# aditya-v-kallappa/FInCFlow

Hardware: AMD Instinct MI355X
Metric: inverse images/sec (+ fwd+logdet ms/img in `forward`), 3x3 conv @64x64x96 (higher is better)
Workload: dtype f32

## Files before the change

### fincflow_amd/csrc/finc_mfma.hip

```cpp
#include "finc_common.h"
#include "finc_tile.h"

#include <stdlib.h>

#include <mutex>
#include <type_traits>
#include <utility>
#include <vector>

namespace {

typedef float v4f __attribute__((ext_vector_type(4)));
typedef unsigned v2u __attribute__((ext_vector_type(2)));
typedef unsigned v4u __attribute__((ext_vector_type(4)));

template <int CQP_, int KH_, int KW_, int NW_ = 1>
struct Cfg {
    static constexpr int CQP = CQP_, KH = KH_, KW = KW_, NW = NW_;
    static constexpr int MTB = CQP / 16;
    static constexpr int NSM = (CQP % 16) / 4;
    static constexpr int MT = MTB + NSM;
    static constexpr int NKZT = CQP / 4;
    static constexpr int NKDT = CQP / 4;
    static_assert(NW == 1 || (NKZT % NW == 0 && NKDT % NW == 0), "K-split must divide the k-steps and the output registers");
// ... 104 lines not shown
    } while (0)
#else
#define FINC_STAMP_AT(k) do { } while (0)
#endif

__device__ unsigned finc_hlp_timeouts = 0;
__device__ unsigned *finc_fault_word = nullptr;
#ifndef FINC_HLP_BUDGET_LOG2
#define FINC_HLP_BUDGET_LOG2 20
#endif
#ifdef FINC_HLP_COUNT
__device__ unsigned finc_hlp_late[2] = {0, 0};
#define FINC_HLP_LATE(k) do { if ((threadIdx.x & 63) == 0) atomicAdd(&finc_hlp_late[k], 1u); } while (0)
extern "C" int finc_debug_hlp_late(unsigned *h) { return (int)hipMemcpyFromSymbol(h, HIP_SYMBOL(finc_hlp_late), 8); }
#else
#define FINC_HLP_LATE(k) do { } while (0)
#endif

constexpr unsigned OFF_INVALID = 0x80000000u;
constexpr unsigned OFF_BAD_CHANNEL = 0x40000000u;

template <int CQP, int KH, int KW, bool SEC, int NW = 1, int NPW = 1, int S64 = 0, int HLP = 0, bool ZPRE = false>
__global__ __launch_bounds__(HLP ? 512 : 64 * NW * NPW) void finc_wave_kernel(const float *__restrict__ in,
                                                            const float *__restrict__ packed, float *__restrict__ out,
                                                            int G, int CQ, int H, int W, int P, int Tend,
                                                            unsigned orient)
{
    using C = Cfg<CQP, KH, KW, NW>;
    constexpr int MT = C::MT, NKZ = C::NKZ, NKD = C::NKD, NK = C::NK, NFRAG = C::NFRAG;
    constexpr int JS = 4 * (KH - 1);
    constexpr int SS = NK * JS;
    extern __shared__ __attribute__((aligned(16))) float lds[];
    static_assert(!HLP || (S64 == 3 && NW == 1 && NPW == 1), "helper waves: the sector-pairing kernel, one compute wave per problem");
    static_assert(!ZPRE || HLP, "premultiplied input: the helper-wave form only");
    const int wvt = (HLP || NW * NPW > 1) ? __builtin_amdgcn_readfirstlane(threadIdx.x >> 6) : 0;
    const bool helper = HLP && wvt >= 4;
    const int wv = HLP ? 0 : wvt % NW;
    const int prob = HLP ? (wvt & 3) : wvt / NW;
    const int lane = threadIdx.x & 63;
    const int q = lane >> 4, p = lane & 15;
    const int bg = blockIdx.x * (HLP ? 4 : NPW) + prob;
    const int g = bg % G;
    const unsigned o = finc_group_orient(orient, g);
    const bool fh = (o & FINC_FLIP_H) != 0, fw = (o & FINC_FLIP_W) != 0;
    const int HW = H * W;
    const unsigned slab_bytes = (unsigned)CQ * (unsigned)HW * 4u;
    const int bg_in = bg, bg_out = bg;
    const __amdgpu_buffer_rsrc_t rin =
        __builtin_amdgcn_make_buffer_rsrc((void *)(in + (size_t)bg_in * CQ * HW), 0, (int)slab_bytes, 0x00020000);
    const __amdgpu_buffer_rsrc_t rout =
        __builtin_amdgcn_make_buffer_rsrc((void *)(out + (size_t)bg_out * CQ * HW), 0, (int)slab_bytes, 0x00020000);
    const int D = W - P + 1;
    const int fifo_n = D * SS;
    const int wave_lds = C::ZRING + C::XRING + fifo_n + SS + 64;
    float *const lds_p = lds + prob * (C::XCH + NW * wave_lds);
    float *xch = lds_p;
    float *zring = lds_p + C::XCH + wv * wave_lds;
    float *xring = zring + C::ZRING;
    auto zcell = [](int qq, int rr) {
        const int lo = ((rr >> 2) ^ ((0x3200 >> (4 * (rr & 3))) & 3)) | ((qq & 1) << 2);
        return lo | (((rr & 3) | ((qq >> 1) << 2)) << 3);
    };
    float *fifo = xring + C::XRING;
    const int trash = fifo_n + lane;
    const unsigned flag_a = (unsigned)(uintptr_t)(lds + 4 * wave_lds + 4 * prob);
    auto flag_set = [flag_a](auto word_c, int v) {
        constexpr int WORD = decltype(word_c)::value;
        (void)flag_a;
#ifdef FINC_HLP_INJECT_TIMEOUT
        if (WORD == 1 && v >= 8) return;
#endif
        if constexpr (HLP) asm volatile("ds_write_b32 %0, %1 offset:%2" ::"v"(flag_a), "v"(v), "n"(4 * WORD) : "memory");
    };
    auto flag_peek = [flag_a](auto word_c, int &reg) {
        constexpr int WORD = decltype(word_c)::value;
        (void)flag_a;
        if constexpr (HLP) asm volatile("ds_read_b32 %0, %1 offset:%2" : "=v"(reg) : "v"(flag_a), "n"(4 * WORD) : "memory");
    };
    auto flag_wait = [flag_a](auto word_c, int target) {
        constexpr int WORD = decltype(word_c)::value;
#ifndef FINC_HLP_NOWAIT
#define FINC_HLP_NOWAIT 0
#endif
        if constexpr (HLP && !((FINC_HLP_NOWAIT >> WORD) & 1)) {
            int budget = 1 << FINC_HLP_BUDGET_LOG2;
            for (; budget > 0; --budget) {
                int v;
                asm volatile("ds_read_b32 %0, %1 offset:%2\n\ts_waitcnt lgkmcnt(0)" : "=v"(v) : "v"(flag_a), "n"(4 * WORD) : "memory");
                if (__builtin_amdgcn_readfirstlane(v) >= target) break;
                __builtin_amdgcn_s_sleep(2);
            }
            if (budget == 0 && (threadIdx.x & 63) == 0) {
                atomicAdd(&finc_hlp_timeouts, 1u);
                if (finc_fault_word) __hip_atomic_store(finc_fault_word, 1u, __ATOMIC_RELAXED, __HIP_MEMORY_SCOPE_SYSTEM);
            }
        }
    };

    constexpr int NSMALL = (NFRAG / MT) * C::NSM, NSR = (NSMALL + 3) / 4;
    float af[NFRAG];
    float afs[NSR > 0 ? NSR : 1];
    constexpr bool PAIR2 = finc_pair2_form<C>(HLP);
    constexpr int NPAIRF = PAIR2 ? C::NPAIR : C::NPAIR1;
    float afp[C::PAIR ? NPAIRF : 1];
    static_assert(!C::PAIR || ((NKZ * C::NSM) % 4 == 0 && (NK * C::NSM) % 4 == 0),
                  "a packed block register must not straddle a paired and an unpaired tap");
    auto small_paired = [](int sfr) {
        const int tapi = sfr < NKZ * C::NSM ? 0 : 1 + (sfr - NKZ * C::NSM) / (NK * (C::NSM > 0 ? C::NSM : 1));
        return C::PAIR && ((tapi >= 1 && tapi <= 4) || (PAIR2 && (tapi == 6 || tapi == 7)));
    };
    if (!helper) {
        const float *pk = packed + (size_t)g * C::NPACK * 64 + lane;
        auto gindex = [&](int f) {
            if (f < NKZ * MT) return (wv * NKZ + f / MT) * MT + f % MT;
            const int ff = f - NKZ * MT;
            return C::NKZT * MT + ((ff / (MT * NKD)) * C::NKDT + wv * NKD + (ff / MT) % NKD) * MT + ff % MT;
        };
#pragma unroll
        for (int f = 0; f < NFRAG; ++f) {
            if (f % MT >= C::MTB) continue;
            if (ZPRE && f < NKZ * MT) { af[f] = 0.f; continue; }
            if (NW == 1 && f < NKZ * MT && finc_zterm_is_zero(C::MTB, f / MT, f % MT)) { af[f] = 0.f; continue; }
            af[f] = pk[gindex(f) * 64];
        }
        const int quad = (lane & 15) >> 2;
#pragma unroll
        for (int r = 0; r < NSR; ++r) {
            if (small_paired(4 * r)) { afs[r] = 0.f; continue; }
            int gi = 0;
#pragma unroll
            for (int a = 3; a >= 0; --a) {
                const int sfr = 4 * r + a < NSMALL ? 4 * r + a : NSMALL - 1;
                constexpr int NSMD = C::NSM > 0 ? C::NSM : 1;
                const int f = (sfr / NSMD) * MT + C::MTB + sfr % NSMD;
                const int ga = gindex(f);
                gi = (a == 3 || quad == a) ? ga : gi;
            }
            afs[r] = pk[gi * 64];
        }
#pragma unroll
        for (int f = 0; f < NFRAG; ++f) {
            if (f % MT >= C::MTB) continue;
            if (ZPRE && f < NKZ * MT) continue;
            if (NW == 1 && f < NKZ * MT && finc_zterm_is_zero(C::MTB, f / MT, f % MT)) continue;
            asm volatile("" : "+a"(af[f]));
        }
#pragma unroll
        for (int r = 0; r < NSR; ++r) {
            if (small_paired(4 * r)) continue;
            asm volatile("" : "+a"(afs[r]));
        }
        if constexpr (C::PAIR) {
            const float *pp = packed + finc_pair_offset(G, C::NPACK, C::NPAIR, g, 0) + lane;
#pragma unroll
            for (int f = 0; f < NPAIRF; ++f) afp[f] = pp[f * 64];
#pragma unroll
            for (int f = 0; f < NPAIRF; ++f) asm volatile("" : "+a"(afp[f]));
        }
    }
    auto mma = [&](v4f &acc_, int f, float b) {
        const int mt = f % MT;
        if (mt < C::MTB) acc_ = __builtin_amdgcn_mfma_f32_16x16x4f32(af[f], b, acc_, 0, 0, 0);
        else {
            const int sfr = (f / MT) * C::NSM + (mt - C::MTB);
            finc_mma_small(acc_, afs[sfr >> 2], b, sfr & 3);
        }
    };
    v4f bias[MT];
    {
        const float *pb = packed + ((size_t)g * C::NPACK + C::NFRAGT + (wv == 0 ? 0 : 4 * MT)) * 64 + lane;
#pragma unroll
        for (int mt = 0; mt < MT; ++mt)
            bias[mt] = (v4f){pb[(4 * mt + 0) * 64], pb[(4 * mt + 1) * 64], pb[(4 * mt + 2) * 64], pb[(4 * mt + 3) * 64]};
    }
    for (int i = lane; i < fifo_n + SS + 64; i += 64) fifo[i] = 0.f;

    const int fl4 = -((p + 3) >> 2);
    const int k0 = fw ? 3 : 0, k1 = fw ? 2 : 1, k2 = fw ? 1 : 2, k3 = fw ? 0 : 3;
    const unsigned lane_t = 4u * (unsigned)q * HW * 4u, lane_b = (unsigned)q * HW * 4u;
    unsigned cmask[NKD];
#pragma unroll
    for (int j = 0; j < NKD; ++j) cmask[j] = chan_d(C::MTB, wv * NKD + j, q) < CQ ? 0u : OFF_BAD_CHANNEL;
    const unsigned zlast = (4 * (wv * NKZ + NKZ - 1) + q) < CQ ? 0u : OFF_BAD_CHANNEL;
    unsigned zpad[NW > 1 ? NKZ : 1];
    if constexpr (NW > 1) {
#pragma unroll
        for (int j = 0; j < NKZ; ++j) zpad[j] = (4 * (wv * NKZ + j) + q) < CQ ? 0u : OFF_BAD_CHANNEL;
    }
    auto zmark = [&](int j) { return NW > 1 ? zpad[j] : (j == NKZ - 1 ? zlast : 0u); };
    const int rowstep = (fh ? -P : P) * W * 4;
    const int dirw = fw ? -1 : 1;

    constexpr unsigned long long PARTNER = 0xCBAFED8943276501ull;
    const int cls = ((p + 3) >> 2) & 1;
    const int part = (int)((PARTNER >> (4 * p)) & 15);
    int srvrow[2], srvhalf[2];
#pragma unroll
    for (int wp = 0; wp < 2; ++wp) {
        const bool own = cls == wp || p >= P;
        srvrow[wp] = own ? p : part;
        srvhalf[wp] = own ? 0 : 1;
    }
    int lcolS[2], lrowS[2], loffS[2], lslotS[2], ldst[2];
    int scolS[2], srowS[2], soffS[2];
#pragma unroll
    for (int wp = 0; wp < 2; ++wp) {
        const int R = srvrow[wp], h = srvhalf[wp];
        const int f = -((R + 3) >> 2);
        lcolS[wp] = 4 * ((wp ? -3 : -4) + 4 + f);
        lrowS[wp] = R;
        lslotS[wp] = ((4 * (((wp ? -3 : -4) + 2 + f + h) % 3 + 3)) % 12);
        ldst[wp] = 4 * zcell(q, R);
        const int c = lcolS[wp] + 4 * h;
        loffS[wp] = ((fh ? H - 1 - R : R) * W + (fw ? W - 4 - c : c)) * 4 + (4 * wv * NKZ + q) * HW * 4;
        scolS[wp] = 4 * ((wp ? -1 : 0) - 2 + f);
        srowS[wp] = R;
        const int sc = scolS[wp] + 4 * h;
        soffS[wp] = ((fh ? H - 1 - R : R) * W + (fw ? W - 4 - sc : sc)) * 4;
    }
    v4u Z[2][NKZ];
#pragma unroll
    for (int wp = 0; wp < 2; ++wp)
#pragma unroll
        for (int j = 0; j < NKZ; ++j) Z[wp][j] = (v4u){0u, 0u, 0u, 0u};
    float XS[2][NKD][4];
#pragma unroll
    for (int wp = 0; wp < 2; ++wp)
#pragma unroll
// ... 73 lines not shown
            if ((FINC_S64_ABLATE & 4) == 0 && phi == 0) {
                const bool ok = lcolS[WP] >= 0 && lrowS[WP] < H && p < P;
                const unsigned vl = ok ? (unsigned)loffS[WP] : OFF_INVALID;
                const unsigned vu = ok ? (unsigned)(loffS[WP] + 32 * dirw) : OFF_INVALID;
#pragma unroll
                for (int j = 0; j < NKZ; ++j) {
                    unsigned ol = j == NKZ - 1 ? vl + zlast : vl, ou = j == NKZ - 1 ? vu + zlast : vu;
                    int so = __builtin_amdgcn_readfirstlane(j * 16 * HW);
                    if constexpr (ZPRE) {
                        const bool tile = j < 4 * C::MTB;
                        const bool last_group = tile ? (C::NSM == 0 && (j >> 2) == C::MTB - 1) : j == C::NKDT - 1;
                        const unsigned add = (tile ? lane_t - lane_b : 0u) + ((last_group && C::CQP != CQ) ? cmask[j] : 0u);
                        ol = vl + add; ou = vu + add;
                        so = __builtin_amdgcn_readfirstlane((tile ? 16 * (j >> 2) + (j & 3) : 16 * C::MTB + 4 * (j - 4 * C::MTB)) * HW * 4);
                    }
                    if constexpr (ZA_AGPR)
                        asm volatile("buffer_load_dwordx4 %0, %1, %2, %3 offen" : "=a"(ZA[WP][j]) : "v"(ol), "s"(rin), "s"(so) : "memory");
                    else
                        asm volatile("buffer_load_dwordx4 %0, %1, %2, %3 offen" : "=v"(Z[WP][j]) : "v"(ol), "s"(rin), "s"(so) : "memory");
                    asm volatile("buffer_load_dwordx4 %0, %1, %2, %3 offen" : "=a"(ZU[WP][j]) : "v"(ou), "s"(rin), "s"(so) : "memory");
                }
            }
            lcolS[WP] += 8;
            loffS[WP] += 32 * dirw;
            if (lcolS[WP] == W) { lcolS[WP] = 0; lrowS[WP] += P; loffS[WP] += rowstep - dirw * W * 4; }
        }
    };

    auto s64_event = [&](auto wp_c, auto vm_c, int pub_b = -0x7fffffff) { s64_part(wp_c, vm_c, pub_b, IC<0>{}); };

    auto sec_event = [&](auto wp_c) {
        constexpr int WP = decltype(wp_c)::value;
        if constexpr (!SEC) return;
        if constexpr (S64L) return;
        float *dst = zring + lslotS[WP] * 64 + ldst[WP];
#pragma unroll
        for (int j = 0; j < NKZ; ++j) *reinterpret_cast<v4u *>(dst + j * C::ZSLOTS * 64) = Z[WP][j];
        lslotS[WP] = lslotS[WP] >= 4 ? lslotS[WP] - 4 : lslotS[WP] + 8;
        const bool ok = lcolS[WP] >= 0 && lrowS[WP] < H && p < P;
        const unsigned vb = ok ? (unsigned)loffS[WP] : OFF_INVALID;
#pragma unroll
        for (int j = 0; j < NKZ; ++j)
            Z[WP][j] = __builtin_amdgcn_raw_buffer_load_b128(rin, (NW > 1 || j == NKZ - 1) ? vb + zmark(j) : vb, j * 16 * HW, 0);
        lcolS[WP] += 8;
        loffS[WP] += 32 * dirw;
        if (lcolS[WP] == W) { lcolS[WP] = 0; lrowS[WP] += P; loffS[WP] += rowstep - dirw * W * 4; }
    };
    auto sec_sread = [&](auto wp_c, int pub_b2 = -0x7fffffff) {
        constexpr int WP = decltype(wp_c)::value;
        if constexpr (!SEC) return;
        if (cls != WP && p < P) {
#pragma unroll
            for (int j = 0; j < NKD; ++j) {
                const float *xo = xring + j * C::XSLOTS * 64, *xp = xring + j * C::XSLOTS * 64;
                XS[WP ^ 1][j][0] = xo[xown[0]];
                XS[WP ^ 1][j][1] = xo[xown[1]];
                XS[WP ^ 1][j][2] = xo[xown[2]];
                XS[WP ^ 1][j][3] = xo[xown[3]];
                XS[WP][j][0] = xp[xprt[0]];
                XS[WP][j][1] = xp[xprt[1]];
                XS[WP][j][2] = xp[xprt[2]];
                XS[WP][j][3] = xp[xprt[3]];
            }
        }
        if constexpr (HLP) {
            if (pub_b2 != -0x7fffffff) {
                asm volatile("s_waitcnt lgkmcnt(0)" ::: "memory");
                flag_set(IC<2>{}, pub_b2);
            }
        }
        const bool ok = scolS[WP] >= 0 && srowS[WP] < H && p < P;
        st_off = ok ? (unsigned)soffS[WP] : OFF_INVALID;
        if constexpr (S64S) {
            const int phi = ((scolS[WP] + 64) >> 3) & 1;
            spark = phi == 0;
            st_off2 = (ok && phi == 1) ? (unsigned)(soffS[WP] - 32 * dirw) : OFF_INVALID;
            if (phi == 0) st_off = OFF_INVALID;
        }
        scolS[WP] += 8;
        soffS[WP] += 32 * dirw;
        if (scolS[WP] == W) { scolS[WP] = 0; srowS[WP] += P; soffS[WP] += rowstep - dirw * W * 4; }
    };
    auto sec_swrite = [&](auto wp_c, int j0, int j1) {
        constexpr int WP = decltype(wp_c)::value;
        if constexpr (!SEC) return;
        const unsigned vt = st_off == OFF_INVALID ? OFF_INVALID : st_off + lane_t;
        const unsigned vb = st_off == OFF_INVALID ? OFF_INVALID : st_off + lane_b;
        const int cpad = C::CQP - CQ;
#pragma unroll
        for (int j = 0; j < NKD; ++j) {
            if (j < j0 || j >= j1) continue;
            const int jj = wv * NKD + j;
            const bool tile = jj < 4 * C::MTB;
            const int uni = __builtin_amdgcn_readfirstlane((tile ? 16 * (jj >> 2) + (jj & 3) : 16 * C::MTB + 4 * (jj - 4 * C::MTB)) * HW * 4);
            unsigned vo = tile ? vt : vb;
            const bool last_group = tile ? (C::NSM == 0 && (jj >> 2) == C::MTB - 1) : jj == C::NKDT - 1;
            if ((NW > 1 || last_group) && cpad != 0) vo += cmask[j];
            v4u v;
            v.x = __builtin_bit_cast(unsigned, XS[WP][j][0]);
            v.y = __builtin_bit_cast(unsigned, XS[WP][j][1]);
            v.z = __builtin_bit_cast(unsigned, XS[WP][j][2]);
            v.w = __builtin_bit_cast(unsigned, XS[WP][j][3]);
            if constexpr (S64S) {
                const unsigned vo2 = st_off2 == OFF_INVALID ? OFF_INVALID : vo - st_off + st_off2;
                if constexpr (PK_AGPR && (!HLP || WP == 0)) {
                    asm volatile("buffer_store_dwordx4 %0, %1, %2, %3 offen" ::"a"(PK[WP][j]), "v"(vo2), "s"(rout), "s"(uni) : "memory");
                } else {
// ... 108 lines not shown
            if constexpr (PH == 1 && !(AB & 2)) io_swrite(0, S1);
            if constexpr (PH == 2) {
                if constexpr (!(AB & 2)) io_swrite(S1, S2);
                if constexpr (!(AB & 4)) io_land();
                if constexpr (!(AB & 1)) io_issue(0, L1, false);
            }
            if constexpr (PH == 3) {
                if constexpr (!(AB & 2)) io_swrite(S2, NKD);
                if constexpr (!(AB & 1)) io_issue(L1, NKZ, true);
            }
        }
    };

    constexpr bool ROT = (KH - 1 + KW) < 6;
    float Q[KH][4][NK];
    float R[KH][KW][NK];
    float DL[KH][KH][NK];
#pragma unroll
    for (int a = 0; a < KH; ++a) {
#pragma unroll
        for (int k = 0; k < 4; ++k)
#pragma unroll
            for (int j = 0; j < NK; ++j) Q[a][k][j] = 0.f;
#pragma unroll
        for (int b = 0; b < KW; ++b)
#pragma unroll
            for (int j = 0; j < NK; ++j) R[a][b][j] = 0.f;
#pragma unroll
        for (int k = 0; k < KH; ++k)
#pragma unroll
            for (int j = 0; j < NK; ++j) DL[a][k][j] = 0.f;
    }
    float fv[KH][NK];
#pragma unroll
    for (int a = 0; a < KH; ++a)
#pragma unroll
        for (int j = 0; j < NK; ++j) fv[a][j] = 0.f;

    const int push_l = p - (P - (KH - 1));
    const bool do_push = KH > 1 && push_l >= 0 && p < P;
    const int push_base = do_push ? q * (KH - 1) + push_l : trash;
    const int push_stride = do_push ? SS : 0;
    int pop_base[KH], pop_stride[KH];
#pragma unroll
    for (int a = 1; a < KH; ++a) {
        pop_base[a] = p < a ? q * (KH - 1) + (KH - 1 - a + p) : trash;
        pop_stride[a] = p < a ? SS : 0;
    }
    int fslot = 0;
    float *push_p = fifo + push_base;
    float *pop_p[KH];
#pragma unroll
    for (int a = 1; a < KH; ++a) pop_p[a] = fifo + pop_base[a] + (D > 1 ? pop_stride[a] : 0);
    auto fifo_push = [&](const float (&v)[NK]) {
#pragma unroll
        for (int j = 0; j < NK; ++j) push_p[j * JS] = v[j];
    };
    auto fifo_pop_all = [&]() {
#pragma unroll
        for (int a = 1; a < KH; ++a) {
#pragma unroll
            for (int j = 0; j < NK; ++j) fv[a][j] = pop_p[a][j * JS];
        }
    };
    auto fifo_advance = [&]() {
        ++fslot;
        push_p += push_stride;
#pragma unroll
        for (int a = 1; a < KH; ++a) pop_p[a] += pop_stride[a];
        if (__builtin_expect(fslot == D, 0)) {
            FINC_COLD();
            fslot = 0;
            push_p = fifo + push_base;
        }
        if (__builtin_expect(fslot + 1 == D, 0)) {
            FINC_COLD();
#pragma unroll
            for (int a = 1; a < KH; ++a) pop_p[a] = fifo + pop_base[a];
        }
    };
    auto shift_all = [&](const float (&src)[NK], auto ph_c) {
        constexpr int PHX = decltype(ph_c)::value;
        if constexpr (KH > 1) {
            float sn[KH][NK];
            ShiftOp<1>::apply(sn[1], fv[1], src);
            if constexpr (KH > 2) ShiftOp<2>::apply(sn[2], fv[2], src);
            if constexpr (KH > 3) ShiftOp<3>::apply(sn[3], fv[3], src);
            if constexpr (KH > 4) ShiftOp<4>::apply(sn[4], fv[4], src);
            if constexpr (KH > 5) ShiftOp<5>::apply(sn[5], fv[5], src);
            if constexpr (KH > 6) ShiftOp<6>::apply(sn[6], fv[6], src);
            if constexpr (ROT) {
#pragma unroll
                for (int a = 1; a < KH; ++a)
#pragma unroll
                    for (int j = 0; j < NK; ++j) Q[a][PHX][j] = sn[a][j];
            } else {
#pragma unroll
                for (int j = 0; j < NK; ++j) R[1][0][j] = sn[1][j];
#pragma unroll
                for (int a = 2; a < KH; ++a) {
#pragma unroll
                    for (int k = a - 2; k >= 1; --k)
#pragma unroll
                        for (int j = 0; j < NK; ++j) DL[a][k][j] = DL[a][k - 1][j];
#pragma unroll
                    for (int j = 0; j < NK; ++j) DL[a][0][j] = sn[a][j];
                }
            }
        }
    };

    if constexpr (HLP) {
        if (!helper) { flag_set(IC<0>{}, 0); flag_set(IC<1>{}, -1); flag_set(IC<2>{}, 0); flag_set(IC<3>{}, 0); }
    }
    __syncthreads();

    if constexpr (HLP) {
        if (helper) {
            s64_init();
            const int wlast = Tend >> 2;
            s64_event(IC<0>{}, IC<0>{});
            s64_event(IC<1>{}, IC<0>{});
            s64_event(IC<0>{}, IC<0>{});
            sec_sread(IC<1>{});
            sec_swrite(IC<1>{}, 0, NKD);
            s64_event(IC<1>{}, IC<0>{}, 0);
            sec_sread(IC<0>{});
            asm volatile("s_waitcnt lgkmcnt(0)" ::: "memory");
            flag_set(IC<2>{}, 1);
            sec_swrite(IC<0>{}, 0, NKD);
            constexpr int VMS = 1 + 2 * NKD + 2 * NKZ + 2 * NKD;
// ... 50 lines not shown
        for (int mt = 0; mt < MT; ++mt) acc[mt] = (v4f){0.f, 0.f, 0.f, 0.f};
        float zqc[C::NSM > 0 ? C::NSM : 1], zqn[C::NSM > 0 ? C::NSM : 1];
#pragma unroll
        for (int sb = 0; sb < (C::NSM > 0 ? C::NSM : 1); ++sb) zqc[sb] = zqn[sb] = 0.f;
        v4f accp = (v4f){0.f, 0.f, 0.f, 0.f};
        v4f accq = (v4f){0.f, 0.f, 0.f, 0.f};
        float cy[2] = {0.f, 0.f};

        auto phase_a = [&](auto pha_c, int j0, int j1) {
            constexpr int PHA = decltype(pha_c)::value;
#pragma unroll
            for (int j = j0; j < j1; ++j)
#pragma unroll
                for (int mt = 0; mt < (C::PAIR ? C::MTB : MT); ++mt) {
                    if constexpr (KW > 1)
                        mma(acc[mt], FT + ((0 * KW + 1 - 1) * NK + j) * MT + mt, ROT ? Q[0][(PHA + 3) & 3][j] : R[0][1][j]);
                    if constexpr (KH > 1)
                        mma(acc[mt], FT + ((1 * KW + 0 - 1) * NK + j) * MT + mt, ROT ? Q[1][(PHA + 3) & 3][j] : R[1][0][j]);
                }
            if constexpr (C::PAIR) {
#pragma unroll
                for (int j = j0; j < j1; ++j) {
                    accp = __builtin_amdgcn_mfma_f32_16x16x4f32(afp[j], Q[0][(PHA + 3) & 3][j], accp, 0, 0, 0);
                    accp = __builtin_amdgcn_mfma_f32_16x16x4f32(afp[NK + j], Q[1][(PHA + 3) & 3][j], accp, 0, 0, 0);
                }
            }
        };

#ifdef FINC_STAMP
        unsigned stamp_acc[40];
#pragma unroll
        for (int i = 0; i < 40; ++i) stamp_acc[i] = 0u;
        unsigned long long stamp_prev = 0;
        bool stamp_on = false;
#endif
        auto step = [&](auto ph_c, auto wp_c) {
            constexpr int PH = decltype(ph_c)::value;
            FINC_STAMP_AT(9);
            std::conditional_t<C::PAIR, int, bool> wrap_state;
            if constexpr (C::PAIR) wrap_state = (tm - P) & ~tm;
            else wrap_state = tm >= 0 && tm < P;
            auto any_wrap = [&]() -> bool {
                if constexpr (C::PAIR) {
                    asm volatile("" : "+s"(wrap_state));
                    return wrap_state < 0;
                } else {
                    return wrap_state;
                }
            };
            const bool any_idle = tp1 < P - 1;
            float zraw[NKZ], zv[NKZ], xpk[NKD];
            float xown[NKD];
            v4f accn[MT];
            if constexpr (HLP && PH == 0) {
                asm volatile("s_waitcnt lgkmcnt(0)" ::: "memory");
                if (__builtin_expect(__builtin_amdgcn_readfirstlane(peek_b) < win, 0)) { FINC_COLD(); FINC_HLP_LATE(0); flag_wait(IC<1>{}, win); }
            }
            if constexpr (HLP && PH == 1) flag_peek(IC<2>{}, peek_b2);
            if constexpr (C::PAIR) {
                float rs[C::NSM];
#pragma unroll
                for (int sb = 0; sb < C::NSM; ++sb) {
                    rs[sb] = finc_block_reduce(acc[C::MTB + sb]);
                    if constexpr (ZPRE) rs[sb] += zqc[sb];
                }
                if constexpr (PAIR2) {
                    accp = accq;
                    accp.x += cy[0] + rs[0];
                    accp.y += cy[1] + rs[1];
                } else {
                    const float c0 = accp.z, c1 = accp.w;
                    accp = (v4f){c0 + rs[0], c1 + rs[1], 0.f, 0.f};
                }
            }

#pragma unroll
            for (int j = 0; j < NKZ; ++j) zraw[j] = FINC_ABLATE >= 3 ? af[j] : zrd[j * C::ZSLOTS * 64];
            if constexpr (!ROT) {
#pragma unroll
                for (int a = 0; a < KH; ++a) {
#pragma unroll
                    for (int b = KW - 1; b >= 1; --b) {
                        if (a + b >= 2) {
#pragma unroll
                            for (int j = 0; j < NK; ++j) R[a][b][j] = R[a][b - 1][j];
                        }
                    }
                    if (a >= 2) {
#pragma unroll
                        for (int j = 0; j < NK; ++j) R[a][0][j] = DL[a][a - 2][j];
                    }
                }
                if (__builtin_expect(any_wrap(), 0)) {
                    FINC_COLD();
                    const bool wrapn = p == tm;
#pragma unroll
                    for (int a = 0; a < KH; ++a)
#pragma unroll
                        for (int b = 1; b < KW; ++b) {
                            if (a + b >= 2) {
#pragma unroll
                                for (int j = 0; j < NK; ++j) R[a][b][j] = wrapn ? 0.f : R[a][b][j];
                            }
                        }
                }
            }
// ... 81 lines not shown

            auto post1 = [&]() {
                if constexpr (FINC_ABLATE >= 2 && NW == 1) {
                    pack_d<C>(acc, xpk);
#pragma unroll
                    for (int j = 0; j < NKD; ++j) asm volatile("" ::"v"(xpk[j]));
                    return;
                }
                if constexpr (C::PAIR) {
#pragma unroll
                    for (int mt = 0; mt < C::MTB; ++mt) {
                        xpk[4 * mt + 0] = acc[mt].x;
                        xpk[4 * mt + 1] = acc[mt].y;
                        xpk[4 * mt + 2] = acc[mt].z;
                        xpk[4 * mt + 3] = acc[mt].w;
                    }
                    xpk[4 * C::MTB + 0] = accp.x;
                    xpk[4 * C::MTB + 1] = accp.y;
                    if constexpr (PAIR2) {
                        cy[0] = accp.z;
                        cy[1] = accp.w;
                    }
                    if (__builtin_expect(any_wrap(), 0)) {
                        FINC_COLD();
                        const bool wrapn = p == tm;
                        const float c0 = accp.z, c1 = accp.w;
                        if constexpr (PAIR2) {
                            cy[0] = wrapn ? 0.f : c0;
                            cy[1] = wrapn ? 0.f : c1;
                        } else {
                            accp.z = wrapn ? 0.f : c0;
                            accp.w = wrapn ? 0.f : c1;
                        }
                    }
                } else if constexpr (NW == 1) {
                    pack_d<C>(acc, xpk);
                    if constexpr (ZPRE) {
#pragma unroll
                        for (int sb = 0; sb < C::NSM; ++sb) xpk[4 * C::MTB + sb] += zqc[sb];
                    }
                } else {
#pragma unroll
                    for (int j = 0; j < NKD; ++j) {
                        float sum = xown[j];
#pragma unroll
                        for (int src = 0; src < NW; ++src)
                            if (src != wv)
                                sum += C::XALIAS ? xring[j * C::XSLOTS * 64 + PH * 64 + xwin]
                                                 : xch[((wv * NW + src) * NKD + j) * 64 + lane];
                        xpk[j] = sum;
                    }
                }
#pragma unroll
                for (int j = 0; j < NKD; ++j) xring[j * C::XSLOTS * 64 + PH * 64 + xwin] = xpk[j];
                if constexpr (KH > 1) {
                    fifo_push(xpk);
                    fifo_pop_all();
                }
                if constexpr (C::PAIR) {
#pragma unroll
                    for (int j = 0; j < NK; ++j) Q[0][PH][j] = xpk[j];
                } else if constexpr (KW > 1) {
                    if (__builtin_expect(any_wrap(), 0)) {
                        FINC_COLD();
                        const bool wrapn = p == tm;
#pragma unroll
                        for (int j = 0; j < NK; ++j) (ROT ? Q[0][PH][j] : R[0][1][j]) = wrapn ? 0.f : xpk[j];
                    } else {
#pragma unroll
                        for (int j = 0; j < NK; ++j) (ROT ? Q[0][PH][j] : R[0][1][j]) = xpk[j];
                    }
                }
            };
            auto post2 = [&]() {
                if constexpr (FINC_ABLATE < 2) shift_all(xpk, ph_c);
                if constexpr (C::PAIR && FINC_ABLATE < 2) {
                    if (__builtin_expect(any_wrap(), 0)) {
                        FINC_COLD();
                        const bool wrapn = p == tm;
#pragma unroll
                        for (int j = 0; j < NK; ++j) Q[0][PH][j] = wrapn ? 0.f : Q[0][PH][j];
                    }
                }
            };

            auto chunk = [&](auto ci_c) {
                constexpr int CI = decltype(ci_c)::value;
                constexpr int a = BT::a_of(CI), b = BT::b_of(CI);
#pragma unroll
                for (int j = 0; j < NK; ++j)
#pragma unroll
                    for (int mt = 0; mt < ((C::PAIR && ((a + b == 2 && a < 2) || (PAIR2 && a == 2 && b < 2))) ? C::MTB : MT); ++mt)
                        mma(accn[mt], FT + ((a * KW + b - 1) * NK + j) * MT + mt, ROT ? Q[a][(PH + 9 - a - b) & 3][j] : R[a][b][j]);
                if constexpr (PAIR2 && a == 2 && b == 0) {
#pragma unroll
                    for (int j = 0; j < NK; ++j)
                        accq = __builtin_amdgcn_mfma_f32_16x16x4f32(afp[2 * NK + j], Q[2][(PH + 7) & 3][j], j == 0 ? (v4f){0.f, 0.f, 0.f, 0.f} : accq, 0, 0, 0);
                }
                if constexpr (CI == 0) {
                    if constexpr (HLP && PH == 1) {
                        asm volatile("s_waitcnt lgkmcnt(0)" ::: "memory");
                        if (__builtin_expect(__builtin_amdgcn_readfirstlane(peek_b2) < win + 1, 0)) { FINC_COLD(); FINC_HLP_LATE(1); flag_wait(IC<2>{}, win + 1); }
                    }
                    post1();
                    if constexpr (HLP && PH == 3) flag_set(IC<0>{}, win + 1);
                }
                if constexpr (!HLP && CI == (NCH > 1 ? 1 : 0)) io_phase(ph_c, wp_c);
                if constexpr (CI == (NCH > 2 ? 2 : NCH - 1)) {
                    post2();
                    if constexpr (HLP && PH == 3) flag_peek(IC<1>{}, peek_b);
                }
                FINC_SB();
                if constexpr (CI < 6) FINC_STAMP_AT(2 + CI);
            };
            if constexpr (NCH == 0) {
                post1();
                io_phase(ph_c, wp_c);
                post2();
                FINC_SB();
            } else {
                [&]<int... I>(std::integer_sequence<int, I...>) { (chunk(IC<I>{}), ...); }
                (std::make_integer_sequence<int, NCH>{});
            }
#pragma unroll
            for (int mt = 0; mt < MT; ++mt) acc[mt] = accn[mt];
            if constexpr (ZPRE) {
#pragma unroll
                for (int sb = 0; sb < C::NSM; ++sb) zqc[sb] = zqn[sb];
            }
            if constexpr (NW > 1) __syncthreads();
            ++tp1;
            ++tm; if (tm == W) tm = 0;
            ++nslot; zrd += zstep[PH];
            if (nslot == 12) { nslot = 0; zrd -= 12 * 64; }
            if constexpr (PH == 3) { xwin ^= 256; ++win; }
            fifo_advance();
            FINC_STAMP_AT(8);
        };

        if constexpr (HLP) {
        } else if constexpr (SEC) {
            sec_sread(IC<1>{});
            sec_swrite(IC<1>{}, 0, NKD);
            sec_event(IC<1>{});
            s64_event(IC<1>{}, IC<0>{});
        } else {
            io_sread();
            io_swrite(0, NKD);
            io_land();
            io_issue(0, NKZ, true);
        }
#pragma unroll
        for (int k = 0; k < 3; ++k) {
            ++tp1; ++tm;
            ++nslot; zrd += zstep[k];
            if (nslot == 12) { nslot = 0; zrd -= 12 * 64; }
            fifo_advance();
        }
        {
            const bool started = p <= tp1;
            flag_wait(IC<1>{}, 0);
            peek_b = 0;
#pragma unroll
            for (int mt = 0; mt < MT; ++mt) {
                const float b0 = bias[mt].x, b1 = bias[mt].y, b2 = bias[mt].z, b3 = bias[mt].w;
                acc[mt] = (v4f){started ? b0 : 0.f, started ? b1 : 0.f, started ? b2 : 0.f, started ? b3 : 0.f};
                if constexpr (ZPRE) acc[mt] = (v4f){0.f, 0.f, 0.f, 0.f};
            }
#pragma unroll
            for (int j = 0; j < NKZ; ++j) {
                const float v = zrd[j * C::ZSLOTS * 64];
                const float zvj = started ? v : 0.f;
                if constexpr (ZPRE) {
                    if (j < 4 * C::MTB) acc[j >> 2][j & 3] = zvj;
                    else zqc[j - 4 * C::MTB] = zvj;
                    continue;
                }
#pragma unroll
                for (int mt = 0; mt < MT; ++mt) {
                    if (NW == 1 && finc_zterm_is_zero(C::MTB, j, mt)) continue;
                    mma(acc[mt], FZ + j * MT + mt, zvj);
                }
            }
            ++tp1; ++tm;
            ++nslot; zrd += zstep[3];
            if (nslot == 12) { nslot = 0; zrd -= 12 * 64; }
            xwin ^= 256;
            fifo_advance();
        }
        for (int t0 = 0; t0 < Tend; t0 += SEC ? 8 : 4) {
#ifdef FINC_STAMP
            stamp_on = t0 >= 64 && t0 < 192;
#endif
            step(IC<0>{}, IC<0>{});
            step(IC<1>{}, IC<0>{});
            step(IC<2>{}, IC<0>{});
            step(IC<3>{}, IC<0>{});
            if constexpr (SEC) {
                step(IC<0>{}, IC<1>{});
                step(IC<1>{}, IC<1>{});
                step(IC<2>{}, IC<1>{});
                step(IC<3>{}, IC<1>{});
            }
        }
        if constexpr (HLP) {
        } else if constexpr (SEC) {
            sec_sread(IC<0>{});
            sec_swrite(IC<0>{}, 0, NKD);
        } else {
            io_sread();
            io_swrite(0, NKD);
        }
#ifdef FINC_STAMP
        if (blockIdx.x == 517 && threadIdx.x == 0) {
#pragma unroll
            for (int i = 0; i < 40; ++i) finc_stamp_buf[i] = stamp_acc[i];
        }
#endif
    }
}

__global__ void pack_kernel(const float *__restrict__ wc, const float *__restrict__ scale,
                            const float *__restrict__ shift, float *__restrict__ packed, int Cq, int KH, int KW, int MT,
                            int NKZ, int NKD, int MTB, int nfrag, int npair)
{
    extern __shared__ __attribute__((aligned(16))) double sm[];
    const int g = blockIdx.x;
    const float *wg = wc + (size_t)g * Cq * Cq * KH * KW;
    const int KK = KH * KW;
    double *Linv = sm;
    const int npack = nfrag + 8 * MT;
    for (int j = threadIdx.x; j < Cq; j += blockDim.x) {
        for (int r = 0; r < Cq; ++r) {
            double s = (r == j) ? 1.0 : 0.0;
            for (int k = j; k < r; ++k) s -= (double)wg[((size_t)r * Cq + k) * KK + (KK - 1)] * Linv[k * Cq + j];
            Linv[r * Cq + j] = (r < j) ? 0.0 : s;
        }
    }
    __syncthreads();
    for (int e = threadIdx.x; e < nfrag * 64; e += blockDim.x) {
        const int lane = e & 63, f = e >> 6;
// ... 248 lines not shown
    size_t bank_offset = 0;
    int tail_images = 0;
    bool zpre = false;
    bool affine = false;
    bool align16 = true;
    FincSplitPlan split{};
};

static InvForm inverse_form(int Cq, int H, int W, int KH, int KW)
{
    if (finc_big_bank(Cq, KH, KW)) return finc_big_supported(Cq, H, W, KH, KW) ? INV_BIG : INV_NONE;
    if (stream_bank(Cq, KH, KW)) return finc_stream_supported(Cq, H, W, KH, KW, true) ? INV_STREAM : INV_NONE;
    if (W % 4 != 0 || W < 4 || H < 1) return INV_NONE;
    const int P = W < 16 ? W : 16;
    if (P < KH - 1) return INV_NONE;
    if (!find_inst(padded_cq(Cq, KH, KW), KH, KW, -1, W))
        return finc_big_wide_bank(Cq, KH, KW) && finc_big_supported(Cq, H, W, KH, KW) ? INV_WIDE : INV_NONE;
    if ((size_t)Cq * H * W * 4 >= ((size_t)1 << 30)) return INV_NONE;
    return INV_TABLE;
}

static InvPlan inverse_plan(const FincShape &s)
{
    InvPlan p;
    p.form = inverse_form(s.Cq, s.H, s.W, s.KH, s.KW);
    if (p.form == INV_NONE) return p;
    p.affine = p.form != INV_BIG && p.form != INV_WIDE;
    if (p.form == INV_WIDE) p.bank_offset = wave_bank_bytes(s.G, s.Cq, s.KH, s.KW);
    if (p.form == INV_BIG || p.form == INV_WIDE) return p;
    p.split = finc_split_plan(s);
    p.align16 = !p.split.takes;
    if (p.form == INV_STREAM) return p;

    const long long problems = (long long)s.B * s.G;
    const int cqp = padded_cq(s.Cq, s.KH, s.KW), P = s.W < 16 ? s.W : 16;
    const Inst *i = find_inst(cqp, s.KH, s.KW, problems, s.W);
    if (!i) return InvPlan{};
    if (i->nw == 1 && i->npw == 1 && problems % 2 == 0) {
        const Inst *k = nullptr;
        if (borrowed_cqp(cqp, s.KH, s.KW) && borrowed_form_wins(problems, lds_bytes(*i, s.W, P)))
            k = pair_inst(borrowed_cqp(cqp, s.KH, s.KW), s.KH, s.KW, s.W);
        if (!k && 4 * lds_bytes(*i, s.W, P) + 64 > 160 * 1024) k = pair_inst(cqp, s.KH, s.KW, s.W);
        if (k) i = k;
    }
    p.inst = i;
    if (p.split.takes) {
        p.form = INV_SPLIT;
        return p;
    }
    if (i == borrowed_inst(s.Cq, s.KH, s.KW))
        p.bank_offset = bank_bytes(bank_inst(s.Cq, s.KH, s.KW), s.G);
    const size_t lds = lds_bytes(*i, s.W, P);
    const bool s64 = s.W % 16 == 0 && i->fn_s64 && !finc_no_s64();
    const bool hlp = s64 && i->fn_hlp && problems % 4 == 0 && 4 * lds + 64 <= 160 * 1024 && !finc_no_hlp();
    p.io = hlp ? 3 : s64 ? 2 : s.W % 8 == 0 ? 1 : 0;
    p.fn = hlp ? i->fn_hlp : s64 ? i->fn_s64 : s.W % 8 == 0 ? i->fn_sec : i->fn;
    p.lds = hlp ? 4 * lds + 64 : lds;
    p.grid = hlp ? s.B * s.G / 4 : s.B * s.G / i->npw;
    p.block = hlp ? 512 : 64 * i->nw * i->npw;

    static const bool no_remainder = finc_env("FINC_NO_REMAINDER_LAUNCH") != nullptr;
    const bool one_wave = i->nw == 1 && i->npw == 1, packed_pair = i->nw == 2 && i->npw == 2;
    if (!no_remainder && (one_wave || packed_pair)) {
        long long n1 = packed_pair ? 2 : hlp ? 4 : (long long)((160 * 1024 - 64) / lds);
        n1 = n1 > 4 ? 4 : n1 < 1 ? 1 : n1;
        const long long round = n1 * 256, r = problems % round;
        if (problems > round && r != 0 && r <= 512 && r % s.G == 0) {
            FincShape tail = s;
            tail.B = (int)(r / s.G);
            const InvPlan t = inverse_plan(tail);
            if (t.form == INV_SPLIT || t.inst != i) p.tail_images = tail.B;
        }
    }
    p.zpre = hlp && i->fn_zpre && p.tail_images == 0;
    return p;
}

bool finc_mfma_supported(int Cq, int H, int W, int KH, int KW) { return inverse_form(Cq, H, W, KH, KW) != INV_NONE; }

int finc_mfma_packed_cqp(int Cq, int KH, int KW)
{
    if (finc_big_bank(Cq, KH, KW)) { int w, l, c; return finc_big_info(FincShape{1, 1, Cq, 16, 16, KH, KW, 0}, &w, &l, &c) ? 0 : c; }
    if (stream_bank(Cq, KH, KW)) { int c = 0; return finc_stream_info(FincShape{1, 1, Cq, 16, 16, KH, KW, 0}, true, &c, nullptr, nullptr) ? 0 : c; }
    return padded_cq(Cq, KH, KW);
}

static std::mutex g_dead_mutex;
static std::vector<std::pair<int, const void *>> g_dead_wide;
static void dead_wide_set(const void *packed, bool dead)
{
    int dev = 0;
    if (hipGetDevice(&dev) != hipSuccess) return;
    std::lock_guard<std::mutex> lk(g_dead_mutex);
    for (size_t i = 0; i < g_dead_wide.size(); ++i)
        if (g_dead_wide[i].first == dev && g_dead_wide[i].second == packed) {
            if (!dead) { g_dead_wide[i] = g_dead_wide.back(); g_dead_wide.pop_back(); }
            return;
        }
    if (dead) g_dead_wide.emplace_back(dev, packed);
}
static bool dead_wide_has(const void *packed)
{
    int dev = 0;
    if (hipGetDevice(&dev) != hipSuccess) return false;
    std::lock_guard<std::mutex> lk(g_dead_mutex);
    for (const auto &e : g_dead_wide)
        if (e.first == dev && e.second == packed) return true;
    return false;
}

// ... 125 lines not shown
```

### fincflow_amd/csrc/finc_tile.h

```cpp
#pragma once
#include <stddef.h>

typedef float finc_v4f __attribute__((ext_vector_type(4)));
typedef unsigned finc_v2u __attribute__((ext_vector_type(2)));

template <int MTB>
__device__ inline void finc_mma(finc_v4f &acc, int mt, float a, float b)
{
    if (mt < MTB) acc = __builtin_amdgcn_mfma_f32_16x16x4f32(a, b, acc, 0, 0, 0);
    else acc = __builtin_amdgcn_mfma_f32_4x4x1f32(a, b, acc, 0, 0, 0);
}

__device__ inline void finc_mma_small(finc_v4f &acc, float a4, float b, int abid)
{
    switch (abid & 3) {
    case 0: acc = __builtin_amdgcn_mfma_f32_4x4x1f32(a4, b, acc, 2, 0, 0); break;
    case 1: acc = __builtin_amdgcn_mfma_f32_4x4x1f32(a4, b, acc, 2, 1, 0); break;
    case 2: acc = __builtin_amdgcn_mfma_f32_4x4x1f32(a4, b, acc, 2, 2, 0); break;
    default: acc = __builtin_amdgcn_mfma_f32_4x4x1f32(a4, b, acc, 2, 3, 0); break;
    }
}

__device__ inline float finc_block_reduce(const finc_v4f &acc)
{
    const float r0 = acc.x, r1 = acc.y, r2 = acc.z, r3 = acc.w;
    const finc_v2u a = __builtin_amdgcn_permlane32_swap(__builtin_bit_cast(unsigned, r0), __builtin_bit_cast(unsigned, r2),
                                                        false, false);
    const finc_v2u b = __builtin_amdgcn_permlane32_swap(__builtin_bit_cast(unsigned, r1), __builtin_bit_cast(unsigned, r3),
                                                        false, false);
    const unsigned a0 = a.x, a1 = a.y, b0 = b.x, b1 = b.y;
    const float s02 = __builtin_bit_cast(float, a0) + __builtin_bit_cast(float, a1);
    const float s13 = __builtin_bit_cast(float, b0) + __builtin_bit_cast(float, b1);
    const finc_v2u c = __builtin_amdgcn_permlane16_swap(__builtin_bit_cast(unsigned, s02), __builtin_bit_cast(unsigned, s13),
                                                        false, false);
    const unsigned c0 = c.x, c1 = c.y;
    return __builtin_bit_cast(float, c0) + __builtin_bit_cast(float, c1);
}

__host__ __device__ constexpr bool finc_zterm_is_zero(int MTB, int j, int mt)
{
    return mt < MTB ? 4 * j > 16 * mt + 15 : 4 * j > 16 * MTB + 4 * (mt - MTB) + 3;
}

__host__ __device__ inline int finc_tile_row(int MTB, int mt, int i)
{
    return mt < MTB ? 16 * mt + i : 16 * MTB + 4 * (mt - MTB) + (i & 3);
}

__host__ __device__ constexpr bool finc_pair_bank(int cqp, int KH, int KW) { return KH == 3 && KW == 3 && cqp > 16 && cqp % 16 == 8; }
__host__ __device__ inline int finc_pair_row(int MTB, int i, int *partner)
{
    const int qq = i >> 2, r = i & 3;
    *partner = r >> 1;
    return 16 * MTB + 4 * (r & 1) + qq;
}
__host__ __device__ inline void finc_pair_elem(int MTB, int NKD, int f, int lane, int *row, int *j, int *q, int *a, int *b)
{
    int partner;
    const int pr = f / NKD;
    *row = finc_pair_row(MTB, lane & 15, &partner);
    *j = f % NKD;
    *q = lane >> 4;
    *a = pr;
    *b = (pr == 0 ? 1 : 0) + partner;
}
__host__ __device__ inline size_t finc_pair_offset(int G, int npack, int npair, int g, int f)
{
    return ((size_t)G * npack + (size_t)g * npair + f) * 64;
}
```

Measured before the change: 635,700.

## Read row-shifted operands from a compact LDS layout in the paired helper path

```diff
diff --git a/fincflow_amd/csrc/finc_mfma.hip b/fincflow_amd/csrc/finc_mfma.hip
--- a/fincflow_amd/csrc/finc_mfma.hip
+++ b/fincflow_amd/csrc/finc_mfma.hip
@@ -180,7 +180,10 @@
         __builtin_amdgcn_make_buffer_rsrc((void *)(out + (size_t)bg_out * CQ * HW), 0, (int)slab_bytes, 0x00020000);
     const int D = W - P + 1;
     const int fifo_n = D * SS;
-    const int wave_lds = C::ZRING + C::XRING + fifo_n + SS + 64;
+    constexpr bool PAIR2 = finc_pair2_form<C>(HLP);
+    static_assert(!PAIR2 || (KH - 1 + KW) < 6, "row shifts from LDS: written for operands that rotate in place");
+    constexpr int XJ = PAIR2 ? finc_ls_jstride(KH) : C::XSLOTS * 64;
+    const int wave_lds = PAIR2 ? C::ZRING + NKD * XJ : C::ZRING + C::XRING + fifo_n + SS + 64;
     float *const lds_p = lds + prob * (C::XCH + NW * wave_lds);
     float *xch = lds_p;
     float *zring = lds_p + C::XCH + wv * wave_lds;
@@ -228,7 +231,6 @@
     constexpr int NSMALL = (NFRAG / MT) * C::NSM, NSR = (NSMALL + 3) / 4;
     float af[NFRAG];
     float afs[NSR > 0 ? NSR : 1];
-    constexpr bool PAIR2 = finc_pair2_form<C>(HLP);
     constexpr int NPAIRF = PAIR2 ? C::NPAIR : C::NPAIR1;
     float afp[C::PAIR ? NPAIRF : 1];
     static_assert(!C::PAIR || ((NKZ * C::NSM) % 4 == 0 && (NK * C::NSM) % 4 == 0),
@@ -301,7 +303,13 @@
         for (int mt = 0; mt < MT; ++mt)
             bias[mt] = (v4f){pb[(4 * mt + 0) * 64], pb[(4 * mt + 1) * 64], pb[(4 * mt + 2) * 64], pb[(4 * mt + 3) * 64]};
     }
-    for (int i = lane; i < fifo_n + SS + 64; i += 64) fifo[i] = 0.f;
+    if constexpr (PAIR2) {
+        for (int i = FINC_LS_XBLOCK + lane; i < XJ; i += 64)
+#pragma unroll
+            for (int j = 0; j < NKD; ++j) xring[j * XJ + i] = 0.f;
+    } else {
+        for (int i = lane; i < fifo_n + SS + 64; i += 64) fifo[i] = 0.f;
+    }
 
     const int fl4 = -((p + 3) >> 2);
     const int k0 = fw ? 3 : 0, k1 = fw ? 2 : 1, k2 = fw ? 1 : 2, k3 = fw ? 0 : 3;
@@ -481,7 +489,7 @@
         if (cls != WP && p < P) {
 #pragma unroll
             for (int j = 0; j < NKD; ++j) {
-                const float *xo = xring + j * C::XSLOTS * 64, *xp = xring + j * C::XSLOTS * 64;
+                const float *xo = xring + j * XJ, *xp = xring + j * XJ;
                 XS[WP ^ 1][j][0] = xo[xown[0]];
                 XS[WP ^ 1][j][1] = xo[xown[1]];
                 XS[WP ^ 1][j][2] = xo[xown[2]];
@@ -696,31 +704,78 @@
     float *pop_p[KH];
 #pragma unroll
     for (int a = 1; a < KH; ++a) pop_p[a] = fifo + pop_base[a] + (D > 1 ? pop_stride[a] : 0);
+    const int ls_slots = D > 1 ? D - 1 : 0x7fffffff;
+    float *rd_p[KH];
+    int rd_step[KH], rd_rew8[KH], rd_rewR[KH], push_rew8 = 0, push_rewR = 0, push_step = 0;
+    if constexpr (PAIR2) {
+        const bool pushes = finc_ls_pushes(KH, P, D, lane);
+        push_p = xring + finc_ls_push(KH, P, D, lane, 4, 0);
+        push_step = finc_ls_step(KH, pushes);
+        push_rew8 = finc_ls_rewind8(pushes);
+        push_rewR = finc_ls_rewindR(KH, D, pushes);
+#pragma unroll
+        for (int a = 1; a < KH; ++a) {
+            const bool pops = finc_ls_pops(a, D, lane);
+            rd_p[a] = xring + finc_ls_src(KH, a, D, lane, 4, 0);
+            rd_step[a] = finc_ls_step(KH, pops);
+            rd_rew8[a] = finc_ls_rewind8(pops);
+            rd_rewR[a] = finc_ls_rewindR(KH, D, pops);
+        }
+    }
     auto fifo_push = [&](const float (&v)[NK]) {
 #pragma unroll
-        for (int j = 0; j < NK; ++j) push_p[j * JS] = v[j];
+        for (int j = 0; j < NK; ++j) push_p[j * (PAIR2 ? XJ : JS)] = v[j];
     };
     auto fifo_pop_all = [&]() {
 #pragma unroll
         for (int a = 1; a < KH; ++a) {
 #pragma unroll
             for (int j = 0; j < NK; ++j) fv[a][j] = pop_p[a][j * JS];
+        }
+    };
+    auto shift_lds = [&](auto ph_c) {
+        constexpr int PHX = decltype(ph_c)::value;
+        if constexpr (PAIR2) {
+#pragma unroll
+            for (int a = 1; a < KH; ++a)
+#pragma unroll
+                for (int j = 0; j < NK; ++j) Q[a][PHX][j] = rd_p[a][j * XJ];
+        }
+    };
+    auto ls_rewind8 = [&]() {
+        if constexpr (PAIR2) {
+            push_p -= push_rew8;
+#pragma unroll
+            for (int a = 1; a < KH; ++a) rd_p[a] -= rd_rew8[a];
         }
     };
     auto fifo_advance = [&]() {
         ++fslot;
-        push_p += push_stride;
-#pragma unroll
-        for (int a = 1; a < KH; ++a) pop_p[a] += pop_stride[a];
-        if (__builtin_expect(fslot == D, 0)) {
-            FINC_COLD();
-            fslot = 0;
-            push_p = fifo + push_base;
-        }
-        if (__builtin_expect(fslot + 1 == D, 0)) {
-            FINC_COLD();
-#pragma unroll
-            for (int a = 1; a < KH; ++a) pop_p[a] = fifo + pop_base[a];
+        if constexpr (PAIR2) {
+            push_p += push_step;
+#pragma unroll
+            for (int a = 1; a < KH; ++a) rd_p[a] += rd_step[a];
+            if (__builtin_expect(fslot == ls_slots, 0)) {
+                FINC_COLD();
+                fslot = 0;
+                push_p -= push_rewR;
+#pragma unroll
+                for (int a = 1; a < KH; ++a) rd_p[a] -= rd_rewR[a];
+            }
+        } else {
+            push_p += push_stride;
+#pragma unroll
+            for (int a = 1; a < KH; ++a) pop_p[a] += pop_stride[a];
+            if (__builtin_expect(fslot == D, 0)) {
+                FINC_COLD();
+                fslot = 0;
+                push_p = fifo + push_base;
+            }
+            if (__builtin_expect(fslot + 1 == D, 0)) {
+                FINC_COLD();
+#pragma unroll
+                for (int a = 1; a < KH; ++a) pop_p[a] = fifo + pop_base[a];
+            }
         }
     };
     auto shift_all = [&](const float (&src)[NK], auto ph_c) {
@@ -877,6 +932,7 @@
             float zraw[NKZ], zv[NKZ], xpk[NKD];
             float xown[NKD];
             v4f accn[MT];
+            if constexpr (PAIR2 && FINC_ABLATE < 2) __builtin_amdgcn_s_waitcnt(0xc07f);
             if constexpr (HLP && PH == 0) {
                 asm volatile("s_waitcnt lgkmcnt(0)" ::: "memory");
                 if (__builtin_expect(__builtin_amdgcn_readfirstlane(peek_b) < win, 0)) { FINC_COLD(); FINC_HLP_LATE(0); flag_wait(IC<1>{}, win); }
@@ -1064,10 +1120,12 @@
                     }
                 }
 #pragma unroll
-                for (int j = 0; j < NKD; ++j) xring[j * C::XSLOTS * 64 + PH * 64 + xwin] = xpk[j];
+                for (int j = 0; j < NKD; ++j) xring[j * XJ + PH * 64 + xwin] = xpk[j];
                 if constexpr (KH > 1) {
-                    fifo_push(xpk);
-                    fifo_pop_all();
+                    if constexpr (!PAIR2) {
+                        fifo_push(xpk);
+                        fifo_pop_all();
+                    }
                 }
                 if constexpr (C::PAIR) {
 #pragma unroll
@@ -1085,7 +1143,14 @@
                 }
             };
             auto post2 = [&]() {
-                if constexpr (FINC_ABLATE < 2) shift_all(xpk, ph_c);
+                if constexpr (FINC_ABLATE < 2) {
+                    if constexpr (PAIR2) {
+                        shift_lds(ph_c);
+                        fifo_push(xpk);
+                    } else {
+                        shift_all(xpk, ph_c);
+                    }
+                }
                 if constexpr (C::PAIR && FINC_ABLATE < 2) {
                     if (__builtin_expect(any_wrap(), 0)) {
                         FINC_COLD();
@@ -1147,6 +1212,7 @@
             if (nslot == 12) { nslot = 0; zrd -= 12 * 64; }
             if constexpr (PH == 3) { xwin ^= 256; ++win; }
             fifo_advance();
+            if constexpr (PAIR2 && PH == 3 && decltype(wp_c)::value == 1) ls_rewind8();
             FINC_STAMP_AT(8);
         };
 
@@ -1199,6 +1265,7 @@
             if (nslot == 12) { nslot = 0; zrd -= 12 * 64; }
             xwin ^= 256;
             fifo_advance();
+            if constexpr (PAIR2) ls_rewind8();
         }
         for (int t0 = 0; t0 < Tend; t0 += SEC ? 8 : 4) {
 #ifdef FINC_STAMP
@@ -1553,10 +1620,13 @@
         p.bank_offset = bank_bytes(bank_inst(s.Cq, s.KH, s.KW), s.G);
     const size_t lds = lds_bytes(*i, s.W, P);
     const bool s64 = s.W % 16 == 0 && i->fn_s64 && !finc_no_s64();
-    const bool hlp = s64 && i->fn_hlp && problems % 4 == 0 && 4 * lds + 64 <= 160 * 1024 && !finc_no_hlp();
+    const bool ls = finc_pair_bank(i->cqp, i->kh, i->kw) && i->nw == 1;
+    const size_t lds_hlp = ls ? sizeof(float) * ((size_t)i->wnkz * 12 * 64 + (size_t)i->wnkd * finc_ls_jstride(i->kh)) : lds;
+    const bool hlp = s64 && i->fn_hlp && problems % 4 == 0 && 4 * lds + 64 <= 160 * 1024 && 4 * lds_hlp + 64 <= 160 * 1024 &&
+                     (!ls || s.W - P + 1 <= FINC_LS_DMAX) && !finc_no_hlp();
     p.io = hlp ? 3 : s64 ? 2 : s.W % 8 == 0 ? 1 : 0;
     p.fn = hlp ? i->fn_hlp : s64 ? i->fn_s64 : s.W % 8 == 0 ? i->fn_sec : i->fn;
-    p.lds = hlp ? 4 * lds + 64 : lds;
+    p.lds = hlp ? 4 * lds_hlp + 64 : lds;
     p.grid = hlp ? s.B * s.G / 4 : s.B * s.G / i->npw;
     p.block = hlp ? 512 : 64 * i->nw * i->npw;
 
diff --git a/fincflow_amd/csrc/finc_tile.h b/fincflow_amd/csrc/finc_tile.h
--- a/fincflow_amd/csrc/finc_tile.h
+++ b/fincflow_amd/csrc/finc_tile.h
@@ -68,3 +68,23 @@
 {
     return ((size_t)G * npack + (size_t)g * npair + f) * 64;
 }
+
+constexpr int FINC_LS_DMAX = 49, FINC_LS_XBLOCK = 8 * 64;
+__host__ __device__ constexpr int finc_ls_js(int KH) { return 4 * (KH - 1); }
+__host__ __device__ constexpr int finc_ls_jstride(int KH) { return FINC_LS_XBLOCK + finc_ls_js(KH) * (FINC_LS_DMAX - 1); }
+__host__ __device__ constexpr int finc_ls_xcell(int slot, int lane) { return slot * 64 + lane; }
+__host__ __device__ constexpr int finc_ls_fifo(int KH, int fslot, int q, int l) { return FINC_LS_XBLOCK + fslot * finc_ls_js(KH) + q * (KH - 1) + l; }
+__host__ __device__ constexpr bool finc_ls_pushes(int KH, int P, int D, int lane) { return D > 1 && (lane & 15) >= P - (KH - 1) && (lane & 15) < P; }
+__host__ __device__ constexpr bool finc_ls_pops(int a, int D, int lane) { return D > 1 && (lane & 15) < a; }
+__host__ __device__ constexpr int finc_ls_push(int KH, int P, int D, int lane, int slot, int fslot)
+{
+    return finc_ls_pushes(KH, P, D, lane) ? finc_ls_fifo(KH, fslot, lane >> 4, (lane & 15) - (P - (KH - 1))) : finc_ls_xcell(slot, lane);
+}
+__host__ __device__ constexpr int finc_ls_src(int KH, int a, int D, int lane, int slot, int fslot)
+{
+    if (finc_ls_pops(a, D, lane)) return finc_ls_fifo(KH, fslot, lane >> 4, KH - 1 - a + (lane & 15));
+    return finc_ls_xcell(slot, (lane & 15) >= a ? lane - a : lane - a + 16);
+}
+__host__ __device__ constexpr int finc_ls_step(int KH, bool fifo) { return fifo ? finc_ls_js(KH) : 64; }
+__host__ __device__ constexpr int finc_ls_rewind8(bool fifo) { return fifo ? 0 : FINC_LS_XBLOCK; }
+__host__ __device__ constexpr int finc_ls_rewindR(int KH, int D, bool fifo) { return fifo ? (D - 1) * finc_ls_js(KH) : 0; }
```

After: 643,600, median of 6. 1.2% higher.
